# LANL-Bioinformatics/KWAGE

Hardware: AMD Instinct MI355X
Metric: G k-mer·sample bit-tests/sec (+ achieved HBM GB/s of the gather kernel in `roofline`) (higher is better)
Workload: dtype u32

## Files before the change

### include/kwage_amd.h

```cpp
#ifndef KWAGE_AMD_H
#define KWAGE_AMD_H

#include <stddef.h>
#include <stdint.h>

#ifdef __cplusplus
extern "C" {
#endif

#define KWAGE_AMD_ABI_VERSION 1

enum {
	KWAGE_OK = 0,
	KWAGE_ERR_ARG = -1,
	KWAGE_ERR_DEVICE = -2,
	KWAGE_ERR_IO = -3,
	KWAGE_ERR_FORMAT = -4,
	KWAGE_ERR_HASH = -5,
	KWAGE_ERR_STATE = -6
};

#define KWAGE_MAX_WORD_LEN 32
#define KWAGE_MIN_NUM_HASH 1
#define KWAGE_MAX_NUM_HASH 5
// ... 7 lines not shown
uint32_t kwage_abi_version(void);

typedef struct kwage_ctx kwage_ctx;

int kwage_device_count(void);
int kwage_init(int device, kwage_ctx **out);
void kwage_shutdown(kwage_ctx *ctx);
int kwage_mem_info(kwage_ctx *ctx, uint64_t *free_bytes, uint64_t *total_bytes);
int kwage_device_fingerprint(kwage_ctx *ctx, char *buf, uint64_t len);
int kwage_sync(kwage_ctx *ctx);

int kwage_ctx_set_tuning(kwage_ctx *ctx, const char *name, int64_t value);
int kwage_ctx_get_tuning(kwage_ctx *ctx, const char *name, int64_t *value);
int kwage_ctx_scratch_nonzero(kwage_ctx *ctx, uint64_t out[5]);
int kwage_ctx_refine_stats(kwage_ctx *ctx, uint64_t out[8]);

typedef struct kwage_group kwage_group;

typedef struct {
	uint32_t kmer_len;
	uint32_t num_hash;
	uint32_t log_2_filter_len;
	int32_t  hash_func;
} kwage_params;

int kwage_group_create(kwage_ctx *ctx, const kwage_params *params, uint64_t column_capacity,
                       kwage_group **out);
void kwage_group_destroy(kwage_group *g);

int kwage_group_create_sparse(kwage_ctx *ctx, const kwage_params *params, uint64_t column_capacity,
// ... 241 lines not shown
```

### kwage_amd/csrc/engine.hip

```cpp
#include <hip/hip_runtime.h>
#include <hip/hip_ext.h>

#include <algorithm>
#include <chrono>
#include <cmath>
#include <cstdio>
#include <cctype>
#include <cstring>
#include <new>
#include <string>
#include <thread>
#include <vector>

#include <unistd.h>

#include "host.hpp"
#include "engine_state.hpp"
#include "kernels.hpp"

using namespace kwage;


struct TuningName { const char *name; int64_t Tuning::*field; };
static const TuningName TUNING_NAMES[] = {
	{"walk", &Tuning::walk}, {"walk_min_rows", &Tuning::walk_min_rows}, {"walk_max_kib", &Tuning::walk_max_kib}, {"walk_min_kib", &Tuning::walk_min_kib}, {"walk_tile_kib", &Tuning::walk_tile_kib},
	 {"walk_waves", &Tuning::walk_waves}, {"walk_one_wg_per_cu", &Tuning::walk_one_wg_per_cu},
	{"walk_bands", &Tuning::walk_bands}, {"walk_bands_min_gib", &Tuning::walk_bands_min_gib},
	{"and_vec", &Tuning::and_vec}, {"and_wide", &Tuning::and_wide}, {"and_wide_min_kib", &Tuning::and_wide_min_kib}, {"narrow", &Tuning::narrow}, {"force_segs", &Tuning::force_segs}, {"scores_form", &Tuning::scores_form},
	{"ee_refine", &Tuning::ee_refine}, {"refine_seg_rows", &Tuning::refine_seg_rows}, {"refine_min_rows", &Tuning::refine_min_rows}, {"refine_max_groups", &Tuning::refine_max_groups}, {"refine_unroll", &Tuning::refine_unroll}, {"refine_list_cap", &Tuning::refine_list_cap}, {"refine_static", &Tuning::refine_static}, {"screen_wpc", &Tuning::screen_wpc}, {"count_screen_wpc", &Tuning::count_screen_wpc}, {"count_screen_min_tiles", &Tuning::count_screen_min_tiles}, {"count_screen_check", &Tuning::count_screen_check}, {"count_trunc", &Tuning::count_trunc},
	{"count_walk", &Tuning::count_walk}, {"count_walk_wpc", &Tuning::count_walk_wpc}, {"count_walk_waves", &Tuning::count_walk_waves},
	{"count_walk_min_rows", &Tuning::count_walk_min_rows},
	{"hit_sort_host", &Tuning::hit_sort_host}, {"hit_copy_piece_kb", &Tuning::hit_copy_piece_kb}, {"shared_table_log2", &Tuning::shared_table_log2},
	{"ext_launch_events", &Tuning::ext_launch_events}, {"group_contiguous", &Tuning::group_contiguous}, {"group_placement_probe", &Tuning::group_placement_probe},
};

namespace kwage {

__global__ __launch_bounds__(KM_THREADS) void kmer_kernel(KmerArgs a)
{
	extern __shared__ __attribute__((aligned(16))) unsigned long long lds_tab[];
	__shared__ uint8_t codes[KM_THREADS + KWAGE_MAX_WORD_LEN];
	__shared__ uint32_t count, tile_base;

	const uint32_t q = a.chunk_q ? a.chunk_q[blockIdx.x] : blockIdx.x;
// ... 33 lines not shown
                                                         const uint32_t *map, uint32_t map_len, unsigned long long *missing, uint32_t wgs_per_query)
{
	const uint32_t q = blockIdx.x / wgs_per_query, part = blockIdx.x % wgs_per_query;
	uint32_t *rq = rows + pos_off[q]*num_hash;
	const uint64_t n = (uint64_t)nkmer[q]*num_hash;
	for(uint64_t e = (uint64_t)part*blockDim.x + threadIdx.x; e < n; e += (uint64_t)wgs_per_query*blockDim.x){
		const uint32_t r = rq[e];
		uint32_t lo = 0, hi = map_len;
		while(lo < hi){
			const uint32_t mid = lo + (hi - lo)/2;
			if(map[mid] < r){ lo = mid + 1; } else { hi = mid; }
		}
		if(lo < map_len && map[lo] == r){ rq[e] = lo; }
		else{ rq[e] = 0; atomicAdd(missing, 1ull); }
	}
}

__global__ __launch_bounds__(SEARCH_THREADS) void and_refine_emit_kernel(SearchArgs a, RefineArgs ra)
{
	constexpr int B = 4;
	__shared__ WaveHitBuf hit_bufs[SEARCH_THREADS/WAVE];
	WaveHitBuf *hbuf = &hit_bufs[threadIdx.x >> 6];
	WaveHitState hst;
	const uint32_t lane = threadIdx.x & (WAVE - 1), l = lane & 7u, g = lane >> 3;
	const uint32_t n_clusters = refine_list_end(ra, 0);
	const uint32_t gw = __builtin_amdgcn_readfirstlane(blockIdx.x*(blockDim.x/WAVE) + (threadIdx.x >> 6));
	const uint32_t nw = gridDim.x*(blockDim.x/WAVE);
	for(uint64_t c0 = gw; c0 < n_clusters; c0 += (uint64_t)B*nw){
		RefineCluster cl[B];
		u32x4 m[B];
// ... 244 lines not shown
			int rc = sl->result.reserve(need);
			if(rc){ return rc; }
		}
		cap = (sl->result.cap - head)/sizeof(kwage_hit);
	}
	char *base = (char*)sl->result.p;
	sl->d_counters = (uint64_t*)base;
	sl->d_nkmer = (uint32_t*)(base + 32);
	sl->d_qthr = (uint32_t*)(base + 32 + 4ull*n);
	sl->d_hits = (kwage_hit*)(base + head);
	sl->hit_cap = cap;
	sl->head_bytes = head;
	return KWAGE_OK;
}

int launch_kmer_stage(Slot *sl, const kwage_params &p, kwage_batch *b, const KmerLayout *L, float threshold,
                      uint32_t *d_rows, uint64_t *d_kmers)
{
	int rc = layout_result(sl, b->n, 0, false);
	if(rc){ return rc; }
	if(L->table_slots){
		if((rc = sl->tables.reserve(L->table_slots*sizeof(uint64_t)))){ return rc; }
		HIP_TRY(hipMemsetAsync(sl->tables.p, 0xFF, L->table_slots*sizeof(uint64_t), sl->stream));
	}
	HIP_TRY(hipMemsetAsync(sl->d_counters, 0, 4*sizeof(uint64_t), sl->stream));
	const KmerStageOut o = {d_rows, d_kmers, sl->d_nkmer, sl->d_qthr, (unsigned long long*)sl->tables.p};
	return launch_kmer_kernels(p, b, L, threshold, (threshold == 1.0f) ? 1 : 0, o, sl->stream);
}

struct StageEvents { hipEvent_t start = nullptr, stop = nullptr; };

#define KW_GATHER_LAUNCH(ge, first, last, kernel, grid, block, lds, stream, ...) \
	hipExtLaunchKernelGGL(kernel, grid, block, (uint32_t)(lds), stream, (first) ? (ge).start : nullptr, (last) ? (ge).stop : nullptr, 0u, __VA_ARGS__)

static const uint32_t WALK_MIN_ROWS_PER_WAVE = 64;
static const uint32_t WALK_WAVES_PER_CU = 8;

uint32_t search_blocks(const SearchArgs &a)
{
	const uint64_t tiles = (uint64_t)a.n_queries*a.segs*a.chunks;
// ... 159 lines not shown
	return KWAGE_OK;
}

uint64_t max_segments(const SearchArgs &a, uint64_t max_segs) { return (a.n_queries > 65535) ? 1 : max_segs; }

int reserve_zeroed(DevBuf &buf, uint64_t bytes, hipStream_t s)
{
	if(bytes <= buf.cap){ return KWAGE_OK; }
	int rc = buf.reserve(bytes);
	if(rc){ return rc; }
	HIP_TRY(hipMemsetAsync(buf.p, 0, buf.cap, s));
	return KWAGE_OK;
}

int refine_setup(Slot *sl, const Tuning &tn, const SearchArgs &a, uint64_t total_rows, uint64_t max_rows, uint32_t max_seg, uint64_t item_bytes, uint64_t unit_bytes,
                 uint64_t tiles, uint64_t screen_waves, uint64_t ncu, hipStream_t gs, RefineSetup *out,
                 uint64_t exact_clusters = 0, uint64_t exact_items = 0, uint64_t exact_units = 0)
{
	int rc;
	RefineArgs &ra = out->ra;
	ra.seg_rows = (uint32_t)std::min<int64_t>(std::max<int64_t>(tn.refine_seg_rows, 8), max_seg);
	ra.seg_rows = (uint32_t)std::max<uint64_t>(ra.seg_rows, (max_rows + 65535)/65536);
	ra.min_rows = (uint32_t)std::max<int64_t>(tn.refine_min_rows, 1);
	ra.max_groups = (uint32_t)std::min<int64_t>(std::max<int64_t>(tn.refine_max_groups, 0), 16);
	uint64_t items = std::min<uint64_t>(std::max<uint64_t>(8ull*a.n_queries, 1u << 16), 1u << 20);
	items = std::max<uint64_t>(std::min<uint64_t>(items, (256ull << 20)/item_bytes), 1024);
	uint64_t units = std::min<uint64_t>(std::max<uint64_t>(32*total_rows/ra.seg_rows, 1u << 18), 1u << 25);
	if(unit_bytes){ units = std::max<uint64_t>(std::min<uint64_t>(units, (512ull << 20)/unit_bytes), 4096); }
	if(tn.refine_list_cap > 0){ items = units = (uint64_t)std::min<int64_t>(tn.refine_list_cap, 1 << 20); }
	uint64_t clusters = items;
	if(exact_units){ clusters = exact_clusters; items = exact_items; units = exact_units; }
	if(exact_units && tn.refine_list_cap > 0){ clusters = items = units = (uint64_t)std::min<int64_t>(tn.refine_list_cap, 1 << 20); }
	const uint64_t tiles_per_wave = (tiles + screen_waves - 1)/std::max<uint64_t>(screen_waves, 1);
	auto list = [&](uint64_t cap, uint64_t stat_max, uint64_t chunk_max) {
		RefineList ls;
		ls.cap = (uint32_t)cap;
		ls.stat = (tn.refine_static && !exact_units) ? (uint32_t)std::min<uint64_t>(stat_max, cap/2/std::max<uint64_t>(screen_waves, 1)) : 0u;
		ls.base = (uint32_t)(ls.stat*screen_waves);
		ls.chunk = exact_units ? 1u : (uint32_t)std::max<uint64_t>(1, std::min<uint64_t>(chunk_max, tiles_per_wave/4));
		return ls;
	};
	ra.lc = list(clusters, 32, 32);
	ra.li = list(items, 64, 64);
	ra.lu = list(units, 256, 256);
	if((rc = sl->ref_counters.reserve(8*sizeof(uint32_t)))){ return rc; }
	if((rc = sl->ref_clusters.reserve(clusters*sizeof(RefineCluster)))){ return rc; }
	if((rc = sl->ref_masks.reserve(items*item_bytes))){ return rc; }
	if((rc = sl->ref_units.reserve(units*sizeof(RefineUnit)))){ return rc; }
	if(unit_bytes && (rc = sl->ref_slab.reserve(units*unit_bytes))){ return rc; }
	ra.counters = (uint32_t*)sl->ref_counters.p;
	ra.clusters = (RefineCluster*)sl->ref_clusters.p;
	ra.masks = (uint32_t*)sl->ref_masks.p;
	ra.units = (RefineUnit*)sl->ref_units.p;
	ra.slab = (uint32_t*)sl->ref_slab.p;
	HIP_TRY(hipMemsetAsync(ra.counters, 0, 8*sizeof(uint32_t), gs));
	sl->ref_base[0] = ra.lc.base; sl->ref_base[1] = ra.li.base; sl->ref_base[2] = ra.lu.base;
	sl->ref_cap[0] = ra.lc.cap; sl->ref_cap[1] = ra.li.cap; sl->ref_cap[2] = ra.lu.cap;
	ra.queue_batch = (uint32_t)std::max<uint64_t>(1, std::min<uint64_t>(16, tiles/(8*std::max<uint64_t>(screen_waves, 1))));
	ra.check_every = (tn.count_screen_check == 16 || tn.count_screen_check == 32 || tn.count_screen_check == 64) ? (uint32_t)tn.count_screen_check : 8u;
	out->refine_wgs = (uint32_t)(ncu*8);
	out->emit_wgs = (uint32_t)(ncu*4);
	return KWAGE_OK;
}

uint32_t count_screen_blocks_per_cu(uint32_t planes, uint32_t nh)
{
	static int cache[3][5] = {};
	const int pi = (planes <= 7) ? 0 : (planes <= 10) ? 1 : 2, ni = (int)std::min(std::max(nh, 1u), 5u) - 1;
	if(cache[pi][ni] == 0){
		int nb = 0;
		hipError_t e = hipErrorUnknown;
#define KWAGE_OCC_NH(P, N) case N: e = hipOccupancyMaxActiveBlocksPerMultiprocessor(&nb, count_screen_kernel<P, N>, SEARCH_THREADS, 0); break;
#define KWAGE_OCC_P(I, P) case I: switch(ni + 1){ KWAGE_OCC_NH(P, 1) KWAGE_OCC_NH(P, 2) KWAGE_OCC_NH(P, 3) KWAGE_OCC_NH(P, 4) default: KWAGE_OCC_NH(P, 5) } break;
		switch(pi){ KWAGE_OCC_P(0, 7) KWAGE_OCC_P(1, 10) default: KWAGE_OCC_P(2, 14) }
#undef KWAGE_OCC_P
#undef KWAGE_OCC_NH
		if(e != hipSuccess || nb <= 0){ (void)hipGetLastError(); nb = 2; }
		cache[pi][ni] = nb;
	}
	return (uint32_t)cache[pi][ni];
}

int launch_search_stage(Slot *sl, kwage_group *g, kwage_batch *b, const KmerLayout *L, float threshold, uint32_t flags,
                        kwage_hit *d_hits, uint64_t cap, unsigned long long *hit_count, hipStream_t gs, const StageEvents &ge)
{
	const Tuning &tn = g->ctx->tune;
	const uint64_t ncu = (uint64_t)std::max(g->ctx->ncu, 1);
	SearchArgs a;
	a.db = g->d_bits;
	a.stride = g->stride;
	a.units_per_row = (uint32_t)(g->stride/16);
	a.valid = g->d_valid;
	a.rows = (const uint32_t*)sl->rows.p;
	a.pos_off = L->d_pos_off;
	a.nkmer = sl->d_nkmer;
// ... 23 lines not shown
			const uint64_t waves = ((uint64_t)a.n_queries + G - 1)/G;
			const dim3 grid((uint32_t)((waves + 3)/4)), block(SEARCH_THREADS);
			const int unroll = (waves < ncu*16) ? 16 : 8;
			snprintf(sl->kernel_name, sizeof(sl->kernel_name), "and_narrow_kernel<%u,%d>", G, unroll);
#define KWAGE_NARROW_CASE(GG) case GG: \
				if(unroll == 16){ KW_GATHER_LAUNCH(ge, true, true, (and_narrow_kernel<GG, 16>), grid, block, 0, gs, a); } \
				else{ KW_GATHER_LAUNCH(ge, true, true, (and_narrow_kernel<GG, 8>), grid, block, 0, gs, a); } break;
			switch(G){
				KWAGE_NARROW_CASE(16) KWAGE_NARROW_CASE(8) KWAGE_NARROW_CASE(4)
				default: KWAGE_NARROW_CASE(2)
			}
#undef KWAGE_NARROW_CASE
			HIP_TRY(hipGetLastError());
			return KWAGE_OK;
		}
		if(a.early_exit && tn.ee_refine && a.units_per_row >= WAVE && tn.force_segs <= 0){
			RefineSetup rs;
			const int vec = (a.units_per_row >= 4*WAVE) ? 2 : 1;
			a.segs = 1;
			a.chunks = (a.units_per_row + WAVE*vec - 1)/(WAVE*vec);
			const uint64_t tiles = (uint64_t)a.n_queries*a.chunks;
			const uint64_t screen_waves = (std::min<uint64_t>(tiles, ncu*(uint64_t)std::max<int64_t>(tn.screen_wpc, 1)) + 3)/4*4;
			if((rc = refine_setup(sl, tn, a, L->total_pos*a.num_hash, L->max_pos*a.num_hash, 1u << 20, 128, 0, tiles, screen_waves, ncu, gs, &rs))){ return rc; }
			const int unroll = (tn.refine_unroll == 16) ? 16 : 8;
			snprintf(sl->kernel_name, sizeof(sl->kernel_name), "and_screen_kernel<%d,8>+refine<%d>", vec, unroll);
			const dim3 grid((uint32_t)(screen_waves/4)), block(SEARCH_THREADS);
			if(vec == 2){ KW_GATHER_LAUNCH(ge, true, false, (and_screen_kernel<2, 8>), grid, block, 0, gs, a, rs.ra); }
			else{ KW_GATHER_LAUNCH(ge, true, false, (and_screen_kernel<1, 8>), grid, block, 0, gs, a, rs.ra); }
			if(unroll == 16){ KW_GATHER_LAUNCH(ge, false, false, (and_refine_kernel<16>), dim3(rs.refine_wgs), block, 0, gs, a, rs.ra); }
			else{ KW_GATHER_LAUNCH(ge, false, false, (and_refine_kernel<8>), dim3(rs.refine_wgs), block, 0, gs, a, rs.ra); }
			KW_GATHER_LAUNCH(ge, false, true, and_refine_emit_kernel, dim3(rs.emit_wgs), block, 0, gs, a, rs.ra);
			HIP_TRY(hipGetLastError());
			return KWAGE_OK;
		}
		const int walk_knob = (int)tn.walk;
		const uint64_t walk_min_rows = (tn.walk_min_rows >= 0) ? (uint64_t)tn.walk_min_rows : (uint64_t)WALK_MIN_ROWS_PER_WAVE*256*WALK_WAVES_PER_CU;
		const uint32_t kib = (a.units_per_row + WAVE - 1)/WAVE;
		const uint32_t walk_max_kib = (uint32_t)std::max<int64_t>(tn.walk_max_kib, 0);
// ... 96 lines not shown
	}
	else{
		a.chunks = (a.units_per_row + WAVE - 1)/WAVE;
		const uint32_t planes = planes_for(L->max_pos);
		const bool narrow = tn.narrow && a.units_per_row <= 32 && a.units_per_row > 8 && a.n_queries >= 64 && planes <= 14;
		if(a.early_exit && tn.ee_refine && !narrow && tn.force_segs <= 0 && a.units_per_row >= WAVE
		   && (uint64_t)a.n_queries*a.chunks >= (uint64_t)std::max<int64_t>(tn.count_screen_min_tiles, 1) && planes <= 14){
			const uint64_t tiles = (uint64_t)a.n_queries*a.chunks;
			uint32_t seg = (uint32_t)std::min<int64_t>(std::max<int64_t>(tn.refine_seg_rows, 8), 120)/8*8;
			int up = 7;
			if(L->max_pos > 8192){ seg = (uint32_t)((L->max_pos + 127)/128 + 7)/8*8; up = 14; }
			const uint64_t wpc = std::min<uint64_t>((uint64_t)std::max<int64_t>(tn.count_screen_wpc, 1), 4ull*count_screen_blocks_per_cu(planes, std::min(a.num_hash, 5u)));
			const uint64_t screen_waves = (std::min<uint64_t>(tiles, ncu*wpc) + 3)/4*4;
			if((rc = check_refine_units(planes, up))){ return rc; }
			RefineSetup rs;
			if((rc = refine_setup(sl, tn, a, L->total_pos, 0, seg, (uint64_t)planes*128, (uint64_t)up*128, tiles, screen_waves, ncu, gs, &rs))){ return rc; }
			rs.ra.seg_rows = seg;
			a.segs = 1;
			snprintf(sl->kernel_name, sizeof(sl->kernel_name), "count_screen_kernel<%u,%u>+refine<%d>", planes, std::min(a.num_hash, 5u), up);
			const dim3 grid((uint32_t)(screen_waves/4)), block(SEARCH_THREADS);
#define KWAGE_CS_NH(P, N) case N: KW_GATHER_LAUNCH(ge, true, false, (count_screen_kernel<P, N>), grid, block, 0, gs, a, rs.ra); break;
#define KWAGE_CS_P(P) case P: switch(std::min(a.num_hash, 5u)){ KWAGE_CS_NH(P, 1) KWAGE_CS_NH(P, 2) KWAGE_CS_NH(P, 3) KWAGE_CS_NH(P, 4) default: KWAGE_CS_NH(P, 5) } break;
			switch(planes){ KWAGE_CS_P(7) KWAGE_CS_P(10) default: KWAGE_CS_P(14) }
#undef KWAGE_CS_P
#undef KWAGE_CS_NH
			launch_count_refine_and_emit(planes, up, a, rs, gs, ge);
			HIP_TRY(hipGetLastError());
			return KWAGE_OK;
		}
		if(a.early_exit && tn.ee_refine && tn.count_trunc && tn.count_walk && !narrow && tn.force_segs <= 0 && a.units_per_row >= WAVE && L->total_pos > 0){
			const uint32_t nq = a.n_queries;
// ... 32 lines not shown
			const int up = (seg <= 120) ? 7 : 14;
			uint64_t units_worst = 0;
			for(uint32_t i = 0; i < nq && seg; ++i){
				const uint64_t rest = (L->h_pos_off[i + 1] - L->h_pos_off[i]) - h_kcut[i];
				units_worst += (uint64_t)a.chunks*8*((rest + seg - 1)/seg);
			}
			const uint64_t tiles = (uint64_t)nq*a.chunks;
			const uint64_t units_cap = std::max<uint64_t>(4096, std::min<uint64_t>(units_worst, (1ull << 30)/((uint64_t)up*128 + sizeof(RefineUnit))));
			if(walked*10 <= L->total_pos*7 && slots*a.num_hash >= min_rows && seg <= 16376 && rest_total > 0 && tiles*8*(uint64_t)tplanes*128 <= (1ull << 30)){
				const uint64_t want_waves = (tn.count_walk_waves > 0) ? std::min<uint64_t>((uint64_t)tn.count_walk_waves, slots)
					: std::max<uint64_t>(1, std::min<uint64_t>(chip_waves, slots*a.num_hash/WALK_MIN_ROWS_PER_WAVE));
				const WalkShape shape = walk_shape(tn, want_waves, ncu);
				const uint64_t waves = (uint64_t)shape.wgs*shape.wg_waves;
				if((rc = check_refine_units(tplanes, up))){ return rc; }
				RefineSetup rs;
				if((rc = refine_setup(sl, tn, a, rest_total, 0, (uint32_t)seg, (uint64_t)tplanes*128, (uint64_t)up*128, tiles, waves, ncu, gs, &rs, tiles, tiles*8, units_cap))){ return rc; }
				rs.ra.seg_rows = (uint32_t)seg;
				if((rc = sl->trunc_dev.reserve(((uint64_t)nq + 1)*sizeof(uint64_t) + (uint64_t)nq*sizeof(uint32_t)))){ return rc; }
				HIP_TRY(hipMemcpyAsync(sl->trunc_dev.p, sl->trunc_host.p, ((uint64_t)nq + 1)*sizeof(uint64_t) + (uint64_t)nq*sizeof(uint32_t), hipMemcpyHostToDevice, gs));
				CountWalkArgs wa;
				wa.total_slots = slots;
				wa.per_wave = (slots + waves - 1)/waves;
				wa.coltiles = a.chunks;
				if((rc = sl->cwalk_slab.reserve(waves*2*tplanes*1024))){ return rc; }
				if((rc = reserve_zeroed(sl->cwalk_arrived, waves*CWALK_LEVELS*sizeof(uint32_t), gs))){ return rc; }
				wa.slab = (uint32_t*)sl->cwalk_slab.p;
				wa.arrived = (uint32_t*)sl->cwalk_arrived.p;
				wa.slot_off = (const uint64_t*)sl->trunc_dev.p;
				wa.kcut = (const uint32_t*)((const uint64_t*)sl->trunc_dev.p + nq + 1);
				a.segs = 1;
				snprintf(sl->kernel_name, sizeof(sl->kernel_name), "count_walk_kernel<%u,%u,trunc>+refine<%d>", tplanes, std::min(a.num_hash, 5u), up);
// ... 90 lines not shown
	float kmer_ms = 0, search_ms = 0;
	uint32_t launches = 0;
	char kernel_name[64] = "";
};

int enqueue_search_and_copy(Slot *sl)
{
	int rc;
	kwage_group *g = sl->g;
	kwage_batch *b = sl->b;
	const bool timing = (sl->flags & KWAGE_SEARCH_TIMING) != 0;
	const bool own = (sl->ext_hits == nullptr && sl->ext_cap == 0);
	const uint64_t cap = own ? sl->hit_cap : sl->ext_cap;
	kwage_hit *d_hits = own ? sl->d_hits : sl->ext_hits;
	if(b->n && g->num_columns){
		hipStream_t gs = g->ctx->gather_stream;
		if(sl->n_runs){ HIP_TRY(hipMemsetAsync(sl->runs.p, 0, sl->n_runs*sizeof(unsigned long long), sl->stream)); }
		HIP_TRY(hipEventRecord(sl->kmer_done, sl->stream));
		HIP_TRY(hipStreamWaitEvent(gs, sl->kmer_done, 0));
		if(sl->append && sl->append_reset){ HIP_TRY(hipMemsetAsync(sl->ext_count, 0, sizeof(uint64_t), gs)); }
		const bool ride = g->ctx->tune.ext_launch_events != 0;
		StageEvents ge;
		if(ride){ ge.start = timing ? sl->ev[2] : nullptr; ge.stop = sl->gather_done; }
		else if(timing){ HIP_TRY(hipEventRecord(sl->ev[2], gs)); }
		unsigned long long *hit_count = sl->append ? (unsigned long long*)sl->ext_count : (unsigned long long*)sl->d_counters;
		if((rc = launch_search_stage(sl, g, b, sl->lay, sl->threshold, sl->flags, d_hits, cap, hit_count, gs, ge))){ return rc; }
		if(!ride){ HIP_TRY(hipEventRecord(sl->gather_done, gs)); }
		HIP_TRY(hipStreamWaitEvent(sl->stream, sl->gather_done, 0));
		++sl->launches;
	}
	else if(sl->append && sl->append_reset){
		hipStream_t gs = g->ctx->gather_stream;
		HIP_TRY(hipMemsetAsync(sl->ext_count, 0, sizeof(uint64_t), gs));
		HIP_TRY(hipEventRecord(sl->gather_done, gs));
		HIP_TRY(hipStreamWaitEvent(sl->stream, sl->gather_done, 0));
	}
	if(sl->append){
		HIP_TRY(hipMemcpyAsync(sl->d_counters, sl->ext_count, sizeof(uint64_t), hipMemcpyDeviceToDevice, sl->stream));
	}
	else if(sl->ext_count){
		HIP_TRY(hipMemcpyAsync(sl->ext_count, sl->d_counters, sizeof(uint64_t), hipMemcpyDeviceToDevice, sl->stream));
	}
	sl->staged_hits = own ? std::min<uint64_t>(SPEC_HITS, cap) : 0;
// ... 24 lines not shown
	if((rc = sl->rows.reserve(std::max<uint64_t>(L->total_pos*g->params.num_hash, 1)*sizeof(uint32_t)))){ return rc; }
	sl->g = g; sl->b = b; sl->lay = L; sl->threshold = threshold; sl->flags = flags;
	sl->ext_hits = ext_hits; sl->ext_cap = ext_cap; sl->ext_count = ext_count;
	sl->append = append; sl->append_reset = append_reset; sl->col_base = col_base;
	sl->launches = 0;
	sl->n_runs = 0;
	sl->runs_per_query = 0;
	if(ext_hits == nullptr && ext_cap == 0 && b->n && g->num_columns){
		const uint64_t kib = (g->stride/16 + WAVE - 1)/WAVE;
		const uint64_t walk_tile = (uint64_t)std::min<int64_t>(std::max<int64_t>(ctx->tune.walk_tile_kib, 1), 16);
		sl->runs_per_query = (uint32_t)(kib + (kib + walk_tile - 1)/walk_tile + 4);
		sl->n_runs = (uint64_t)b->n*sl->runs_per_query;
		if((rc = sl->runs.reserve(sl->n_runs*sizeof(unsigned long long)))){ return rc; }
	}

	const bool timing_kmer = (flags & KWAGE_SEARCH_TIMING) && (flags & KWAGE_SEARCH_TIMING_KMER);
	if(timing_kmer){ HIP_TRY(hipEventRecord(sl->ev[0], sl->stream)); }
	if((rc = launch_kmer_stage(sl, g->params, b, L, threshold, (uint32_t*)sl->rows.p, nullptr))){ return rc; }
	if(g->d_row_map && b->n){
		if((rc = launch_remap_rows(g, b->n, L, (uint32_t*)sl->rows.p, sl->d_nkmer, (unsigned long long*)sl->d_counters + 2, sl->stream))){ return rc; }
	}
	if(timing_kmer){ HIP_TRY(hipEventRecord(sl->ev[1], sl->stream)); }
	if((rc = enqueue_search_and_copy(sl))){ return rc; }
	sl->busy = true;
	return KWAGE_OK;
}

int collect_search_steps(Slot *sl, SearchOutcome *out);

int collect_search(Slot *sl, SearchOutcome *out)
{
	if(!sl->busy){ return fail(KWAGE_ERR_STATE, "no pending search in this slot"); }
	kwage_ctx *ctx = sl->g->ctx;
// ... 18 lines not shown
	sl->busy = false;
	while(true){
		HIP_TRY(hipStreamSynchronize(sl->stream));
		const uint64_t *hc = (const uint64_t*)sl->h_stage.p;
		if(hc[2] != 0){
			return fail(KWAGE_ERR_STATE, "%llu row indices of this batch are not among the rows of the sparse group (it was created for other queries)",
			            (unsigned long long)hc[2]);
		}
		out->n_hits = hc[0];
		out->total_kmers = 0;
		const uint32_t *hn = (const uint32_t*)((const char*)sl->h_stage.p + 32);
		for(uint32_t i = 0; i < sl->b->n; ++i){ out->total_kmers += hn[i]; }
		const uint64_t cap = own ? sl->hit_cap : sl->ext_cap;
		if(!own || out->n_hits <= cap){ break; }
		if((rc = layout_result(sl, sl->b->n, out->n_hits, true))){ return rc; }
		HIP_TRY(hipMemsetAsync(sl->d_counters, 0, sizeof(uint64_t), sl->stream));
		if((rc = enqueue_search_and_copy(sl))){ return rc; }
	}
	out->staged_hits = sl->staged_hits;
	out->launches = sl->launches;
	memcpy(out->kernel_name, sl->kernel_name, sizeof(out->kernel_name));
	if(timing_kmer){ HIP_TRY(hipEventElapsedTime(&out->kmer_ms, sl->ev[0], sl->ev[1])); }
	if(timing && sl->launches){ HIP_TRY(hipEventElapsedTime(&out->search_ms, sl->ev[2], sl->gather_done)); }
	return KWAGE_OK;
}

Slot *free_slot(kwage_ctx *ctx)
{
	for(int i = 0; i < 2; ++i){ if(!ctx->slot[i].busy){ return &ctx->slot[i]; } }
	return nullptr;
}
// ... 70 lines not shown
	if(e == hipSuccess){ e = hipMemcpyAsync(h, d, sizeof(h), hipMemcpyDeviceToHost, ctx->stream); }
	if(e == hipSuccess){ e = hipStreamSynchronize(ctx->stream); }
	(void)hipFree(d);
	if(e != hipSuccess){ return fail(KWAGE_ERR_DEVICE, "kwage_ctx_scratch_nonzero: %s", hipGetErrorString(e)); }
	for(int j = 0; j < 5; ++j){ out[j] = h[j]; }
	return KWAGE_OK;
}

extern "C" int kwage_ctx_refine_stats(kwage_ctx *ctx, uint64_t out[8])
{
	if(!ctx || !out){ return fail(KWAGE_ERR_ARG, "kwage_ctx_refine_stats: NULL argument"); }
	for(int i = 0; i < 2; ++i){ if(ctx->slot[i].busy){ return fail(KWAGE_ERR_STATE, "kwage_ctx_refine_stats: a search is pending on this context"); } }
	int rc = set_device(ctx);
	if(rc){ return rc; }
	HIP_TRY(hipStreamSynchronize(ctx->gather_stream));
	for(int k = 0; k < 2; ++k){
		Slot *sl = &ctx->slot[k];
		uint32_t h[4] = {0, 0, 0, 0};
		if(sl->ref_counters.p){ HIP_TRY(hipMemcpy(h, sl->ref_counters.p, sizeof(h), hipMemcpyDeviceToHost)); }
		for(int j = 0; j < 3; ++j){ out[4*k + j] = std::min<uint64_t>((uint64_t)sl->ref_base[j] + h[j], sl->ref_cap[j]); }
		out[4*k + 3] = sl->ref_cap[2];
	}
	return KWAGE_OK;
}

namespace kwage {
hipStream_t ctx_stream(kwage_ctx *ctx) { return ctx->stream; }
int ctx_device(kwage_ctx *ctx) { return ctx->device; }
}

extern "C" int kwage_device_count(void)
{
	int n = 0;
	if(hipGetDeviceCount(&n) != hipSuccess){ return 0; }
	return n;
}

// ... 480 lines not shown
extern "C" int kwage_hash_batch(kwage_ctx *ctx, const kwage_params *params, kwage_batch *b,
                                uint64_t *kmer_offsets, uint32_t *num_query_kmer, uint64_t *kmers, uint32_t *rows)
{
	if(!ctx || !params || !b || !kmer_offsets || !num_query_kmer){ return fail(KWAGE_ERR_ARG, "kwage_hash_batch: NULL argument"); }
	int rc = check_params(params);
	if(rc){ return rc; }
	if(b->ctx != ctx){ return fail(KWAGE_ERR_ARG, "kwage_hash_batch: batch belongs to another context"); }
	if((rc = set_device(ctx))){ return rc; }
	Slot *sl = &ctx->slot[0];
	if(sl->busy){ return fail(KWAGE_ERR_STATE, "kwage_hash_batch: a search is pending on this context"); }
	const KmerLayout *L = nullptr;
	if((rc = batch_prepare(b, params->kmer_len, &L))){ return rc; }
	const uint64_t np = std::max<uint64_t>(L->total_pos, 1);
	if((rc = sl->rows.reserve(np*params->num_hash*sizeof(uint32_t)))){ return rc; }
	if((rc = ctx->kmers.reserve(np*sizeof(uint64_t)))){ return rc; }
	if((rc = launch_kmer_stage(sl, *params, b, L, 1.0f, (uint32_t*)sl->rows.p, (uint64_t*)ctx->kmers.p))){ return rc; }
	memcpy(kmer_offsets, L->h_pos_off.data(), ((size_t)b->n + 1)*sizeof(uint64_t));
	if(b->n){ HIP_TRY(hipMemcpyAsync(num_query_kmer, sl->d_nkmer, (size_t)b->n*sizeof(uint32_t), hipMemcpyDeviceToHost, ctx->stream)); }
	if(kmers && L->total_pos){ HIP_TRY(hipMemcpyAsync(kmers, ctx->kmers.p, L->total_pos*sizeof(uint64_t), hipMemcpyDeviceToHost, ctx->stream)); }
	if(rows && L->total_pos){ HIP_TRY(hipMemcpyAsync(rows, sl->rows.p, L->total_pos*params->num_hash*sizeof(uint32_t), hipMemcpyDeviceToHost, ctx->stream)); }
	HIP_TRY(hipStreamSynchronize(ctx->stream));
	return KWAGE_OK;
}

namespace {

int run_shared_kmer_pass(kwage_ctx *ctx, const kwage_params &p, kwage_batch *b, uint32_t *d_bloom_bits, uint64_t *distinct)
{
	Slot *sl = &ctx->slot[0];
	if(sl->busy){ return fail(KWAGE_ERR_STATE, "a search is pending on this context"); }
	const KmerLayout *L = nullptr;
// ... 102 lines not shown
```

### kwage_amd/csrc/engine_state.hpp

```cpp
#ifndef KWAGE_AMD_ENGINE_STATE_HPP
#define KWAGE_AMD_ENGINE_STATE_HPP

#include <hip/hip_runtime.h>

#include <algorithm>
#include <deque>
#include <memory>
#include <mutex>
#include <vector>

#include "internal.h"

#define HIP_TRY(expr)                                                                          \
	do {                                                                                       \
		hipError_t _e = (expr);                                                                \
		if(_e != hipSuccess){                                                                  \
			return fail(KWAGE_ERR_DEVICE, "%s failed: %s (%s:%d)", #expr, hipGetErrorString(_e), \
			            __FILE__, __LINE__);                                                   \
		}                                                                                      \
	} while(0)

struct kwage_group;
struct kwage_batch;
struct kwage_ctx;
// ... 163 lines not shown
	void close()
	{
		std::lock_guard<std::mutex> lock(mu);
		open = false;
		for(PinBuf &c : cached){ c.release(); }
		cached.clear();
	}
};


struct Slot {
	hipStream_t stream = nullptr;
	hipEvent_t ev[4] = {nullptr, nullptr, nullptr, nullptr};
	hipEvent_t kmer_done = nullptr;
	hipEvent_t gather_done = nullptr;
	DevBuf rows, tables, partial;
	DevBuf result;
	uint64_t *d_counters = nullptr;
	uint32_t *d_nkmer = nullptr, *d_qthr = nullptr;
	kwage_hit *d_hits = nullptr;
	uint64_t hit_cap = 0, head_bytes = 0;
	PinBuf h_stage;
	DevBuf sort_scratch;
	DevBuf runs;
	uint64_t n_runs = 0;
	uint32_t runs_per_query = 0;
	bool busy = false;
	kwage_group *g = nullptr;
	kwage_batch *b = nullptr;
	const KmerLayout *lay = nullptr;
// ... 21 lines not shown
	int64_t walk_min_rows = -1;
	int64_t walk_max_kib = 16;
	int64_t walk_tile_kib = 16;
	int64_t walk_min_kib = 2;
	int64_t walk_waves = 0;
	int64_t walk_one_wg_per_cu = 1;
	int64_t walk_bands = -1;
	int64_t walk_bands_min_gib = 48;
	int64_t and_vec = 0;
	int64_t and_wide_min_kib = 16;
	int64_t and_wide = 1;
	int64_t narrow = 1;
	int64_t force_segs = 0;
	int64_t scores_form = 0;
	int64_t ee_refine = 1;
	int64_t refine_seg_rows = 32;
	int64_t refine_min_rows = 32;
	int64_t refine_max_groups = 4;
	int64_t refine_unroll = 8;
	int64_t screen_wpc = 20;
	int64_t count_screen_wpc = 32;
	int64_t count_screen_min_tiles = 8192;
	int64_t count_trunc = 1;
	int64_t count_screen_check = 8;
	int64_t refine_static = 1;
	int64_t refine_list_cap = 0;
	int64_t count_walk = 1;
	int64_t count_walk_wpc = 8;
	int64_t count_walk_waves = 0;
	int64_t count_walk_min_rows = -1;
// ... 140 lines not shown
```

### kwage_amd/engine.py

```python
from __future__ import annotations

import ctypes as C
from dataclasses import dataclass
from typing import List, Sequence, Tuple

import numpy as np

from . import native
from .native import Params, check, lib

SEARCH_EARLY_EXIT = 1
SEARCH_TIMING = 2
SEARCH_TIMING_KMER = 4

TOPK_MAX = native.TOPK_MAX

HIT_DTYPE = np.dtype([("query", "<u4"), ("column", "<u4"), ("num_match", "<u4")])


class Context:

    def __init__(self, device: int = 0):
        self._h = C.c_void_p()
        check(lib().kwage_init(device, C.byref(self._h)))
# ... 32 lines not shown

    def get_tuning(self, name: str) -> int:
        v = C.c_int64()
        check(lib().kwage_ctx_get_tuning(self._h, name.encode(), C.byref(v)))
        return int(v.value)

    def scratch_nonzero(self) -> dict:
        out = (C.c_uint64 * 5)()
        check(lib().kwage_ctx_scratch_nonzero(self._h, out))
        return dict(zip(("walk_or", "walk_done", "band_or", "band_state", "cwalk_arrived"), (int(x) for x in out)))

    def refine_stats(self) -> list:
        out = (C.c_uint64 * 8)()
        check(lib().kwage_ctx_refine_stats(self._h, out))
        return [dict(zip(("clusters", "items", "units", "units_cap"), (int(x) for x in out[4 * k:4 * k + 4]))) for k in range(2)]

    def tuning(self, **knobs):
        ctx = self

        class _Scope:
            def __enter__(self):
                self.old = {k: ctx.get_tuning(k) for k in knobs}
                for k, v in knobs.items():
                    ctx.set_tuning(k, v)
                return ctx

            def __exit__(self, *exc):
                for k, v in self.old.items():
                    ctx.set_tuning(k, v)
        return _Scope()
# ... 633 lines not shown
```

### kwage_amd/native.py

```python
from __future__ import annotations

import ctypes as C
import os
import subprocess

_HERE = os.path.dirname(os.path.abspath(__file__))
_CSRC = os.path.join(_HERE, "csrc")
_LIB = os.path.join(_HERE, "lib", "libkwage_amd.so")
KWAGE_BIN = os.path.join(_HERE, "bin", "kwage")
KWAGE_DBTOOL_BIN = os.path.join(_HERE, "bin", "kwage_dbtool")
KWAGE_TOP_BIN = os.path.join(_HERE, "bin", "kwage_top")
KWAGE_TOP_NODE_BIN = os.path.join(_HERE, "bin", "kwage_top_node")
KWAGE_SCORES_BIN = os.path.join(_HERE, "bin", "kwage_scores")
KWAGE_NEAR_BIN = os.path.join(_HERE, "bin", "kwage_near")
TOPK_MAX = 1024


class KwageError(RuntimeError):
    def __init__(self, code: int, msg: str):
        super().__init__("kwage_amd error %d: %s" % (code, msg))
        self.code = code
        self.message = msg


# ... 66 lines not shown
_SIGNATURES = [
    ("kwage_last_error", C.c_char_p, []),
    ("kwage_abi_version", C.c_uint32, []),
    ("kwage_device_count", C.c_int, []),
    ("kwage_init", C.c_int, [C.c_int, C.POINTER(_P)]),
    ("kwage_shutdown", None, [_P]),
    ("kwage_mem_info", C.c_int, [_P, C.POINTER(C.c_uint64), C.POINTER(C.c_uint64)]),
    ("kwage_device_fingerprint", C.c_int, [_P, C.c_char_p, C.c_uint64]),
    ("kwage_set_load_progress", None, [_P, C.POINTER(C.c_uint64)]),
    ("kwage_sort_hits", None, [C.c_void_p, C.c_uint64]),
    ("kwage_sync", C.c_int, [_P]),
    ("kwage_ctx_set_tuning", C.c_int, [_P, C.c_char_p, C.c_int64]),
    ("kwage_ctx_get_tuning", C.c_int, [_P, C.c_char_p, C.POINTER(C.c_int64)]),
    ("kwage_ctx_scratch_nonzero", C.c_int, [_P, C.POINTER(C.c_uint64)]),
    ("kwage_ctx_refine_stats", C.c_int, [_P, C.POINTER(C.c_uint64)]),
    ("kwage_group_create", C.c_int, [_P, C.POINTER(Params), C.c_uint64, C.POINTER(_P)]),
    ("kwage_group_destroy", None, [_P]),
    ("kwage_group_create_sparse", C.c_int, [_P, C.POINTER(Params), C.c_uint64, _P, C.c_uint64, C.POINTER(_P)]),
    ("kwage_group_add_columns", C.c_int, [_P, _P, C.c_uint64, C.c_uint32, C.POINTER(C.c_uint64)]),
    ("kwage_group_add_db_file", C.c_int, [_P, C.c_char_p, C.POINTER(C.c_uint64), C.POINTER(C.c_uint32)]),
    ("kwage_group_add_db_files", C.c_int, [_P, C.POINTER(C.c_char_p), C.c_uint32, C.POINTER(C.c_uint64), C.POINTER(C.c_uint32)]),
    ("kwage_group_add_random_columns", C.c_int, [_P, C.c_uint64, C.c_uint64, C.c_uint32, C.POINTER(C.c_uint64)]),
    ("kwage_group_set_bits", C.c_int, [_P, _P, _P, C.c_uint64]),
    ("kwage_group_read_rows", C.c_int, [_P, _P, C.c_uint64, _P, C.c_uint64]),
    ("kwage_group_finalize", C.c_int, [_P]),
    ("kwage_group_num_columns", C.c_uint64, [_P]),
    ("kwage_group_column_span", C.c_uint64, [_P]),
    ("kwage_group_row_bytes", C.c_uint64, [_P]),
    ("kwage_group_row_stride", C.c_uint64, [_P]),
    ("kwage_group_device_bytes", C.c_uint64, [_P]),
# ... 107 lines not shown
```

Measured before the change: 50570.

## Run small early-exit search stages on the slot's own stream and fuse clears

Adds a routing decision so that small early-exit AND-screen searches launch their gather stage on the slot's own stream instead of the shared gather stream. This removes the cross-stream event record/wait pair, which lets the two slots' searches overlap rather than serialising on the shared gather queue. It also replaces several hipMemsetAsync calls (counters, runs, refine counters) with a single clear kernel launched at the kmer stage, cutting per-search launch overhead. In exchange, refine counters must now be reserved earlier, and concurrent gathers may contend for GPU resources.

```diff
diff --git a/include/kwage_amd.h b/include/kwage_amd.h
--- a/include/kwage_amd.h
+++ b/include/kwage_amd.h
@@ -45,6 +45,7 @@
 int kwage_ctx_get_tuning(kwage_ctx *ctx, const char *name, int64_t *value);
 int kwage_ctx_scratch_nonzero(kwage_ctx *ctx, uint64_t out[5]);
 int kwage_ctx_refine_stats(kwage_ctx *ctx, uint64_t out[8]);
+int kwage_ctx_stage_routes(kwage_ctx *ctx, uint64_t out[2]);
 
 typedef struct kwage_group kwage_group;
 
diff --git a/kwage_amd/csrc/engine.hip b/kwage_amd/csrc/engine.hip
--- a/kwage_amd/csrc/engine.hip
+++ b/kwage_amd/csrc/engine.hip
@@ -27,7 +27,7 @@
 	 {"walk_waves", &Tuning::walk_waves}, {"walk_one_wg_per_cu", &Tuning::walk_one_wg_per_cu},
 	{"walk_bands", &Tuning::walk_bands}, {"walk_bands_min_gib", &Tuning::walk_bands_min_gib},
 	{"and_vec", &Tuning::and_vec}, {"and_wide", &Tuning::and_wide}, {"and_wide_min_kib", &Tuning::and_wide_min_kib}, {"narrow", &Tuning::narrow}, {"force_segs", &Tuning::force_segs}, {"scores_form", &Tuning::scores_form},
-	{"ee_refine", &Tuning::ee_refine}, {"refine_seg_rows", &Tuning::refine_seg_rows}, {"refine_min_rows", &Tuning::refine_min_rows}, {"refine_max_groups", &Tuning::refine_max_groups}, {"refine_unroll", &Tuning::refine_unroll}, {"refine_list_cap", &Tuning::refine_list_cap}, {"refine_static", &Tuning::refine_static}, {"screen_wpc", &Tuning::screen_wpc}, {"count_screen_wpc", &Tuning::count_screen_wpc}, {"count_screen_min_tiles", &Tuning::count_screen_min_tiles}, {"count_screen_check", &Tuning::count_screen_check}, {"count_trunc", &Tuning::count_trunc},
+	{"ee_refine", &Tuning::ee_refine}, {"ee_overlap", &Tuning::ee_overlap}, {"ee_overlap_tiles_per_wave", &Tuning::ee_overlap_tiles_per_wave}, {"refine_seg_rows", &Tuning::refine_seg_rows}, {"refine_min_rows", &Tuning::refine_min_rows}, {"refine_max_groups", &Tuning::refine_max_groups}, {"refine_unroll", &Tuning::refine_unroll}, {"refine_list_cap", &Tuning::refine_list_cap}, {"refine_static", &Tuning::refine_static}, {"screen_wpc", &Tuning::screen_wpc}, {"count_screen_wpc", &Tuning::count_screen_wpc}, {"count_screen_min_tiles", &Tuning::count_screen_min_tiles}, {"count_screen_check", &Tuning::count_screen_check}, {"count_trunc", &Tuning::count_trunc},
 	{"count_walk", &Tuning::count_walk}, {"count_walk_wpc", &Tuning::count_walk_wpc}, {"count_walk_waves", &Tuning::count_walk_waves},
 	{"count_walk_min_rows", &Tuning::count_walk_min_rows},
 	{"hit_sort_host", &Tuning::hit_sort_host}, {"hit_copy_piece_kb", &Tuning::hit_copy_piece_kb}, {"shared_table_log2", &Tuning::shared_table_log2},
@@ -91,6 +91,15 @@
 		if(lo < map_len && map[lo] == r){ rq[e] = lo; }
 		else{ rq[e] = 0; atomicAdd(missing, 1ull); }
 	}
+}
+
+__global__ __launch_bounds__(256) void search_clear_kernel(unsigned long long *counters, uint32_t counter_words, unsigned long long *runs, uint64_t n_runs,
+                                                           uint32_t *ref_counters)
+{
+	const uint64_t i0 = (uint64_t)blockIdx.x*blockDim.x + threadIdx.x;
+	if(i0 < counter_words){ counters[i0] = 0; }
+	if(ref_counters && i0 < 8){ ref_counters[i0] = 0; }
+	for(uint64_t i = i0; i < n_runs; i += (uint64_t)gridDim.x*blockDim.x){ runs[i] = 0; }
 }
 
 __global__ __launch_bounds__(SEARCH_THREADS) void and_refine_emit_kernel(SearchArgs a, RefineArgs ra)
@@ -365,8 +374,25 @@
 	return KWAGE_OK;
 }
 
+int launch_search_clear(Slot *sl, uint32_t counter_words, bool lists)
+{
+	uint32_t *ref = nullptr;
+	uint64_t n_runs = 0;
+	if(lists){
+		int rc = sl->ref_counters.reserve(8*sizeof(uint32_t));
+		if(rc){ return rc; }
+		ref = (uint32_t*)sl->ref_counters.p;
+		n_runs = sl->n_runs;
+	}
+	const uint32_t wgs = (uint32_t)std::max<uint64_t>(1, std::min<uint64_t>(1024, (n_runs + 255)/256));
+	hipLaunchKernelGGL(search_clear_kernel, dim3(wgs), dim3(256), 0, sl->stream, (unsigned long long*)sl->d_counters, counter_words,
+	                   (unsigned long long*)sl->runs.p, n_runs, ref);
+	HIP_TRY(hipGetLastError());
+	return KWAGE_OK;
+}
+
 int launch_kmer_stage(Slot *sl, const kwage_params &p, kwage_batch *b, const KmerLayout *L, float threshold,
-                      uint32_t *d_rows, uint64_t *d_kmers)
+                      uint32_t *d_rows, uint64_t *d_kmers, bool search)
 {
 	int rc = layout_result(sl, b->n, 0, false);
 	if(rc){ return rc; }
@@ -374,7 +400,7 @@
 		if((rc = sl->tables.reserve(L->table_slots*sizeof(uint64_t)))){ return rc; }
 		HIP_TRY(hipMemsetAsync(sl->tables.p, 0xFF, L->table_slots*sizeof(uint64_t), sl->stream));
 	}
-	HIP_TRY(hipMemsetAsync(sl->d_counters, 0, 4*sizeof(uint64_t), sl->stream));
+	if((rc = launch_search_clear(sl, 4, search))){ return rc; }
 	const KmerStageOut o = {d_rows, d_kmers, sl->d_nkmer, sl->d_qthr, (unsigned long long*)sl->tables.p};
 	return launch_kmer_kernels(p, b, L, threshold, (threshold == 1.0f) ? 1 : 0, o, sl->stream);
 }
@@ -564,7 +590,7 @@
 }
 
 int refine_setup(Slot *sl, const Tuning &tn, const SearchArgs &a, uint64_t total_rows, uint64_t max_rows, uint32_t max_seg, uint64_t item_bytes, uint64_t unit_bytes,
-                 uint64_t tiles, uint64_t screen_waves, uint64_t ncu, hipStream_t gs, RefineSetup *out,
+                 uint64_t tiles, uint64_t screen_waves, uint64_t ncu, RefineSetup *out,
                  uint64_t exact_clusters = 0, uint64_t exact_items = 0, uint64_t exact_units = 0)
 {
 	int rc;
@@ -593,7 +619,7 @@
 	ra.lc = list(clusters, 32, 32);
 	ra.li = list(items, 64, 64);
 	ra.lu = list(units, 256, 256);
-	if((rc = sl->ref_counters.reserve(8*sizeof(uint32_t)))){ return rc; }
+	if(!sl->ref_counters.p){ return fail(KWAGE_ERR_STATE, "refine counters were not reserved by the search's clear launch"); }
 	if((rc = sl->ref_clusters.reserve(clusters*sizeof(RefineCluster)))){ return rc; }
 	if((rc = sl->ref_masks.reserve(items*item_bytes))){ return rc; }
 	if((rc = sl->ref_units.reserve(units*sizeof(RefineUnit)))){ return rc; }
@@ -603,7 +629,6 @@
 	ra.masks = (uint32_t*)sl->ref_masks.p;
 	ra.units = (RefineUnit*)sl->ref_units.p;
 	ra.slab = (uint32_t*)sl->ref_slab.p;
-	HIP_TRY(hipMemsetAsync(ra.counters, 0, 8*sizeof(uint32_t), gs));
 	sl->ref_base[0] = ra.lc.base; sl->ref_base[1] = ra.li.base; sl->ref_base[2] = ra.lu.base;
 	sl->ref_cap[0] = ra.lc.cap; sl->ref_cap[1] = ra.li.cap; sl->ref_cap[2] = ra.lu.cap;
 	ra.queue_batch = (uint32_t)std::max<uint64_t>(1, std::min<uint64_t>(16, tiles/(8*std::max<uint64_t>(screen_waves, 1))));
@@ -629,6 +654,28 @@
 		cache[pi][ni] = nb;
 	}
 	return (uint32_t)cache[pi][ni];
+}
+
+struct ScreenPlan { bool use; int vec; uint32_t chunks; uint64_t tiles, screen_waves; };
+
+ScreenPlan plan_and_screen(const Tuning &tn, const kwage_group *g, uint32_t n_queries, float threshold, uint32_t flags, uint64_t ncu)
+{
+	ScreenPlan p = {false, 1, 0, 0, 0};
+	const uint32_t units_per_row = (uint32_t)(g->stride/16);
+	if(threshold != 1.0f || !(flags & KWAGE_SEARCH_EARLY_EXIT) || !tn.ee_refine || units_per_row < WAVE || tn.force_segs > 0){ return p; }
+	p.use = true;
+	p.vec = (units_per_row >= 4*WAVE) ? 2 : 1;
+	p.chunks = (units_per_row + WAVE*p.vec - 1)/(WAVE*p.vec);
+	p.tiles = (uint64_t)n_queries*p.chunks;
+	p.screen_waves = (std::min<uint64_t>(p.tiles, ncu*(uint64_t)std::max<int64_t>(tn.screen_wpc, 1)) + 3)/4*4;
+	return p;
+}
+
+bool stage_on_own_stream(const Tuning &tn, const kwage_group *g, const kwage_batch *b, float threshold, uint32_t flags, bool append, uint64_t ncu)
+{
+	if(!tn.ee_overlap || append || !b->n || !g->num_columns){ return false; }
+	const ScreenPlan p = plan_and_screen(tn, g, b->n, threshold, flags, ncu);
+	return p.use && p.tiles <= (uint64_t)std::max<int64_t>(tn.ee_overlap_tiles_per_wave, 0)*p.screen_waves;
 }
 
 int launch_search_stage(Slot *sl, kwage_group *g, kwage_batch *b, const KmerLayout *L, float threshold, uint32_t flags,
@@ -682,14 +729,14 @@
 			HIP_TRY(hipGetLastError());
 			return KWAGE_OK;
 		}
-		if(a.early_exit && tn.ee_refine && a.units_per_row >= WAVE && tn.force_segs <= 0){
+		const ScreenPlan sp = plan_and_screen(tn, g, a.n_queries, threshold, flags, ncu);
+		if(sp.use){
 			RefineSetup rs;
-			const int vec = (a.units_per_row >= 4*WAVE) ? 2 : 1;
+			const int vec = sp.vec;
 			a.segs = 1;
-			a.chunks = (a.units_per_row + WAVE*vec - 1)/(WAVE*vec);
-			const uint64_t tiles = (uint64_t)a.n_queries*a.chunks;
-			const uint64_t screen_waves = (std::min<uint64_t>(tiles, ncu*(uint64_t)std::max<int64_t>(tn.screen_wpc, 1)) + 3)/4*4;
-			if((rc = refine_setup(sl, tn, a, L->total_pos*a.num_hash, L->max_pos*a.num_hash, 1u << 20, 128, 0, tiles, screen_waves, ncu, gs, &rs))){ return rc; }
+			a.chunks = sp.chunks;
+			const uint64_t tiles = sp.tiles, screen_waves = sp.screen_waves;
+			if((rc = refine_setup(sl, tn, a, L->total_pos*a.num_hash, L->max_pos*a.num_hash, 1u << 20, 128, 0, tiles, screen_waves, ncu, &rs))){ return rc; }
 			const int unroll = (tn.refine_unroll == 16) ? 16 : 8;
 			snprintf(sl->kernel_name, sizeof(sl->kernel_name), "and_screen_kernel<%d,8>+refine<%d>", vec, unroll);
 			const dim3 grid((uint32_t)(screen_waves/4)), block(SEARCH_THREADS);
@@ -816,7 +863,7 @@
 			const uint64_t screen_waves = (std::min<uint64_t>(tiles, ncu*wpc) + 3)/4*4;
 			if((rc = check_refine_units(planes, up))){ return rc; }
 			RefineSetup rs;
-			if((rc = refine_setup(sl, tn, a, L->total_pos, 0, seg, (uint64_t)planes*128, (uint64_t)up*128, tiles, screen_waves, ncu, gs, &rs))){ return rc; }
+			if((rc = refine_setup(sl, tn, a, L->total_pos, 0, seg, (uint64_t)planes*128, (uint64_t)up*128, tiles, screen_waves, ncu, &rs))){ return rc; }
 			rs.ra.seg_rows = seg;
 			a.segs = 1;
 			snprintf(sl->kernel_name, sizeof(sl->kernel_name), "count_screen_kernel<%u,%u>+refine<%d>", planes, std::min(a.num_hash, 5u), up);
@@ -879,7 +926,7 @@
 				const uint64_t waves = (uint64_t)shape.wgs*shape.wg_waves;
 				if((rc = check_refine_units(tplanes, up))){ return rc; }
 				RefineSetup rs;
-				if((rc = refine_setup(sl, tn, a, rest_total, 0, (uint32_t)seg, (uint64_t)tplanes*128, (uint64_t)up*128, tiles, waves, ncu, gs, &rs, tiles, tiles*8, units_cap))){ return rc; }
+				if((rc = refine_setup(sl, tn, a, rest_total, 0, (uint32_t)seg, (uint64_t)tplanes*128, (uint64_t)up*128, tiles, waves, ncu, &rs, tiles, tiles*8, units_cap))){ return rc; }
 				rs.ra.seg_rows = (uint32_t)seg;
 				if((rc = sl->trunc_dev.reserve(((uint64_t)nq + 1)*sizeof(uint64_t) + (uint64_t)nq*sizeof(uint32_t)))){ return rc; }
 				HIP_TRY(hipMemcpyAsync(sl->trunc_dev.p, sl->trunc_host.p, ((uint64_t)nq + 1)*sizeof(uint64_t) + (uint64_t)nq*sizeof(uint32_t), hipMemcpyHostToDevice, gs));
@@ -1000,10 +1047,12 @@
 	const uint64_t cap = own ? sl->hit_cap : sl->ext_cap;
 	kwage_hit *d_hits = own ? sl->d_hits : sl->ext_hits;
 	if(b->n && g->num_columns){
-		hipStream_t gs = g->ctx->gather_stream;
-		if(sl->n_runs){ HIP_TRY(hipMemsetAsync(sl->runs.p, 0, sl->n_runs*sizeof(unsigned long long), sl->stream)); }
-		HIP_TRY(hipEventRecord(sl->kmer_done, sl->stream));
-		HIP_TRY(hipStreamWaitEvent(gs, sl->kmer_done, 0));
+		const bool own_route = sl->own_route;
+		hipStream_t gs = own_route ? sl->stream : g->ctx->gather_stream;
+		if(!own_route){
+			HIP_TRY(hipEventRecord(sl->kmer_done, sl->stream));
+			HIP_TRY(hipStreamWaitEvent(gs, sl->kmer_done, 0));
+		}
 		if(sl->append && sl->append_reset){ HIP_TRY(hipMemsetAsync(sl->ext_count, 0, sizeof(uint64_t), gs)); }
 		const bool ride = g->ctx->tune.ext_launch_events != 0;
 		StageEvents ge;
@@ -1012,7 +1061,7 @@
 		unsigned long long *hit_count = sl->append ? (unsigned long long*)sl->ext_count : (unsigned long long*)sl->d_counters;
 		if((rc = launch_search_stage(sl, g, b, sl->lay, sl->threshold, sl->flags, d_hits, cap, hit_count, gs, ge))){ return rc; }
 		if(!ride){ HIP_TRY(hipEventRecord(sl->gather_done, gs)); }
-		HIP_TRY(hipStreamWaitEvent(sl->stream, sl->gather_done, 0));
+		if(!own_route){ HIP_TRY(hipStreamWaitEvent(sl->stream, sl->gather_done, 0)); }
 		++sl->launches;
 	}
 	else if(sl->append && sl->append_reset){
@@ -1067,9 +1116,11 @@
 		if((rc = sl->runs.reserve(sl->n_runs*sizeof(unsigned long long)))){ return rc; }
 	}
 
+	sl->own_route = stage_on_own_stream(ctx->tune, g, b, threshold, flags, append, (uint64_t)std::max(ctx->ncu, 1));
+
 	const bool timing_kmer = (flags & KWAGE_SEARCH_TIMING) && (flags & KWAGE_SEARCH_TIMING_KMER);
 	if(timing_kmer){ HIP_TRY(hipEventRecord(sl->ev[0], sl->stream)); }
-	if((rc = launch_kmer_stage(sl, g->params, b, L, threshold, (uint32_t*)sl->rows.p, nullptr))){ return rc; }
+	if((rc = launch_kmer_stage(sl, g->params, b, L, threshold, (uint32_t*)sl->rows.p, nullptr, true))){ return rc; }
 	if(g->d_row_map && b->n){
 		if((rc = launch_remap_rows(g, b->n, L, (uint32_t*)sl->rows.p, sl->d_nkmer, (unsigned long long*)sl->d_counters + 2, sl->stream))){ return rc; }
 	}
@@ -1118,7 +1169,7 @@
 		const uint64_t cap = own ? sl->hit_cap : sl->ext_cap;
 		if(!own || out->n_hits <= cap){ break; }
 		if((rc = layout_result(sl, sl->b->n, out->n_hits, true))){ return rc; }
-		HIP_TRY(hipMemsetAsync(sl->d_counters, 0, sizeof(uint64_t), sl->stream));
+		if((rc = launch_search_clear(sl, 1, true))){ return rc; }
 		if((rc = enqueue_search_and_copy(sl))){ return rc; }
 	}
 	out->staged_hits = sl->staged_hits;
@@ -1219,6 +1270,8 @@
 	int rc = set_device(ctx);
 	if(rc){ return rc; }
 	HIP_TRY(hipStreamSynchronize(ctx->gather_stream));
+	HIP_TRY(hipStreamSynchronize(ctx->slot[0].stream));
+	HIP_TRY(hipStreamSynchronize(ctx->slot[1].stream));
 	for(int k = 0; k < 2; ++k){
 		Slot *sl = &ctx->slot[k];
 		uint32_t h[4] = {0, 0, 0, 0};
@@ -1226,6 +1279,14 @@
 		for(int j = 0; j < 3; ++j){ out[4*k + j] = std::min<uint64_t>((uint64_t)sl->ref_base[j] + h[j], sl->ref_cap[j]); }
 		out[4*k + 3] = sl->ref_cap[2];
 	}
+	return KWAGE_OK;
+}
+
+extern "C" int kwage_ctx_stage_routes(kwage_ctx *ctx, uint64_t out[2])
+{
+	if(!ctx || !out){ return fail(KWAGE_ERR_ARG, "kwage_ctx_stage_routes: NULL argument"); }
+	for(int i = 0; i < 2; ++i){ if(ctx->slot[i].busy){ return fail(KWAGE_ERR_STATE, "kwage_ctx_stage_routes: a search is pending on this context"); } }
+	for(int k = 0; k < 2; ++k){ out[k] = ctx->slot[k].own_route ? 1 : 0; }
 	return KWAGE_OK;
 }
 
@@ -1736,7 +1797,7 @@
 	const uint64_t np = std::max<uint64_t>(L->total_pos, 1);
 	if((rc = sl->rows.reserve(np*params->num_hash*sizeof(uint32_t)))){ return rc; }
 	if((rc = ctx->kmers.reserve(np*sizeof(uint64_t)))){ return rc; }
-	if((rc = launch_kmer_stage(sl, *params, b, L, 1.0f, (uint32_t*)sl->rows.p, (uint64_t*)ctx->kmers.p))){ return rc; }
+	if((rc = launch_kmer_stage(sl, *params, b, L, 1.0f, (uint32_t*)sl->rows.p, (uint64_t*)ctx->kmers.p, false))){ return rc; }
 	memcpy(kmer_offsets, L->h_pos_off.data(), ((size_t)b->n + 1)*sizeof(uint64_t));
 	if(b->n){ HIP_TRY(hipMemcpyAsync(num_query_kmer, sl->d_nkmer, (size_t)b->n*sizeof(uint32_t), hipMemcpyDeviceToHost, ctx->stream)); }
 	if(kmers && L->total_pos){ HIP_TRY(hipMemcpyAsync(kmers, ctx->kmers.p, L->total_pos*sizeof(uint64_t), hipMemcpyDeviceToHost, ctx->stream)); }
diff --git a/kwage_amd/csrc/engine_state.hpp b/kwage_amd/csrc/engine_state.hpp
--- a/kwage_amd/csrc/engine_state.hpp
+++ b/kwage_amd/csrc/engine_state.hpp
@@ -201,6 +201,7 @@
 	hipEvent_t ev[4] = {nullptr, nullptr, nullptr, nullptr};
 	hipEvent_t kmer_done = nullptr;
 	hipEvent_t gather_done = nullptr;
+	bool own_route = false;
 	DevBuf rows, tables, partial;
 	DevBuf result;
 	uint64_t *d_counters = nullptr;
@@ -252,6 +253,8 @@
 	int64_t force_segs = 0;
 	int64_t scores_form = 0;
 	int64_t ee_refine = 1;
+	int64_t ee_overlap = 1;
+	int64_t ee_overlap_tiles_per_wave = 4;
 	int64_t refine_seg_rows = 32;
 	int64_t refine_min_rows = 32;
 	int64_t refine_max_groups = 4;
diff --git a/kwage_amd/engine.py b/kwage_amd/engine.py
--- a/kwage_amd/engine.py
+++ b/kwage_amd/engine.py
@@ -70,6 +70,11 @@
         out = (C.c_uint64 * 8)()
         check(lib().kwage_ctx_refine_stats(self._h, out))
         return [dict(zip(("clusters", "items", "units", "units_cap"), (int(x) for x in out[4 * k:4 * k + 4]))) for k in range(2)]
+
+    def stage_routes(self) -> list:
+        out = (C.c_uint64 * 2)()
+        check(lib().kwage_ctx_stage_routes(self._h, out))
+        return [int(x) for x in out]
 
     def tuning(self, **knobs):
         ctx = self
diff --git a/kwage_amd/native.py b/kwage_amd/native.py
--- a/kwage_amd/native.py
+++ b/kwage_amd/native.py
@@ -104,6 +104,7 @@
     ("kwage_ctx_get_tuning", C.c_int, [_P, C.c_char_p, C.POINTER(C.c_int64)]),
     ("kwage_ctx_scratch_nonzero", C.c_int, [_P, C.POINTER(C.c_uint64)]),
     ("kwage_ctx_refine_stats", C.c_int, [_P, C.POINTER(C.c_uint64)]),
+    ("kwage_ctx_stage_routes", C.c_int, [_P, C.POINTER(C.c_uint64)]),
     ("kwage_group_create", C.c_int, [_P, C.POINTER(Params), C.c_uint64, C.POINTER(_P)]),
     ("kwage_group_destroy", None, [_P]),
     ("kwage_group_create_sparse", C.c_int, [_P, C.POINTER(Params), C.c_uint64, _P, C.c_uint64, C.POINTER(_P)]),
```

After: 50230. Within noise of the previous version (-0.7%).
